# cics-nd/gptorch

Hardware: AMD Instinct MI355X
Metric: GP log-marginal-likelihood evals/sec (Cholesky+solve) at NxD fp64 (higher is better)
Workload: dtype f64; 1 GPU; C3: GPR+Matern52 N=32768 D=16 fp64 LML eval; N=32768, D=16, dy=1, kernel=Matern52, parallelism=1 GPU

## Files before the change

### gptorch_amd/_native.py

```python
import ctypes
import os

_HERE = os.path.dirname(os.path.abspath(__file__))
LIB_PATH = os.environ.get("GPN_LIB", os.path.join(_HERE, "lib", "libgpnative.so"))

c_void_p, c_int, c_int64, c_double = ctypes.c_void_p, ctypes.c_int, ctypes.c_int64, ctypes.c_double

SIGNATURES = {
    "gpn_version": (c_int, []),
    "gpn_arch": (ctypes.c_char_p, []),
    "gpn_last_hip_error": (ctypes.c_char_p, []),
    "gpn_factor_ld": (c_int64, [c_int64, c_int64]),
    "gpn_factor_rows": (c_int64, [c_int64, c_int64]),
    "gpn_winv_bytes": (c_int64, [c_int64]),
    "gpn_kernel_matrix": (c_int, [c_void_p, c_int, c_void_p, c_int64, c_void_p, c_int64, c_int,
                                  c_void_p, c_void_p, c_int, c_void_p, c_int, c_void_p, c_int64]),
    "gpn_pack_rhs": (c_int, [c_void_p, c_void_p, c_void_p, c_int64, c_int, c_void_p, c_int64]),
    "gpn_potrf_lower": (c_int, [c_void_p, c_void_p, c_int64, c_int64, c_int64, c_void_p, c_void_p]),
    "gpn_potrf_lower_panel": (c_int, [c_void_p, c_void_p, c_int64, c_int64, c_int64, c_void_p, c_void_p]),
    "gpn_potrf_lower_batched": (c_int, [c_void_p, c_void_p, c_int64, c_int64, c_int64, c_int64, c_void_p, c_int64, c_void_p, c_int]),
    "gpn_lml_reduce_batched": (c_int, [c_void_p, c_void_p, c_int64, c_int64, c_int64, c_int64, c_void_p, c_int]),
    "gpn_lml_forward_batched": (c_int, [c_void_p, c_int, c_int, c_void_p, c_int64, c_int64, c_int, c_void_p, c_int64, c_void_p, c_int64, c_int,
                                        c_void_p, c_void_p, c_int, c_void_p, c_void_p, c_int64, c_int64, c_void_p, c_int64, c_void_p, c_void_p]),
    "gpn_potrf_panel_width": (c_int64, [c_int64]),
    "gpn_potrf_panel_levels": (c_int, [c_int64, c_void_p]),
    "gpn_potrf_lower_persistent": (c_int, [c_void_p, c_void_p, c_int64, c_int64, c_int64, c_void_p, c_void_p]),
    "gpn_potrf_persistent_supported": (c_int, [c_int64, c_int64]),
    "gpn_potrf_persistent_plan": (c_int, [c_int64, c_int64, c_void_p, c_void_p, c_int64, c_void_p, c_int64]),
    "gpn_release_stream": (c_int, [c_void_p]),
    "gpn_trtri_diag": (c_int, [c_void_p, c_void_p, c_int64, c_int64, c_void_p, c_void_p]),
    "gpn_trsm_right_lt": (c_int, [c_void_p, c_void_p, c_int64, c_int64, c_void_p, c_void_p, c_int64, c_int64]),
    "gpn_lml_reduce": (c_int, [c_void_p, c_void_p, c_int64, c_int64, c_int64, c_void_p]),
    "gpn_gemm_nt": (c_int, [c_void_p, c_int64, c_int64, c_int64, c_double, c_void_p, c_int64,
                            c_void_p, c_int64, c_double, c_void_p, c_int64, c_int, c_int]),
    "gpn_gemm_nt_stair": (c_int, [c_void_p, c_int64, c_int64, c_int64, c_int64, c_double, c_void_p, c_int64,
                                  c_void_p, c_int64, c_double, c_void_p, c_int64, c_int64, c_int]),
    "gpn_gemm_nt_batched": (c_int, [c_void_p, c_int64, c_int64, c_int64, c_double, c_void_p, c_int64, c_int64,
                                    c_void_p, c_int64, c_int64, c_double, c_void_p, c_int64, c_int64, c_int, c_int, c_int]),
    "gpn_gemm_nt_batched_scaled": (c_int, [c_void_p, c_int64, c_int64, c_int64, c_void_p, c_void_p, c_int64, c_int64,
                                           c_void_p, c_int64, c_int64, c_double, c_void_p, c_int64, c_int64, c_int, c_int, c_int]),
    "gpn_kernel_matrix_batched": (c_int, [c_void_p, c_int, c_int, c_void_p, c_int64, c_int64, c_void_p, c_int64, c_int64, c_int,
                                          c_void_p, c_void_p, c_int, c_void_p, c_int, c_void_p, c_int64, c_int64]),
    "gpn_trsm_right_lt_batched": (c_int, [c_void_p, c_void_p, c_int64, c_int64, c_int64, c_void_p, c_int64,
                                          c_void_p, c_int64, c_int64, c_int64, c_int]),
    "gpn_trtri_upper_batched": (c_int, [c_void_p, c_void_p, c_int64, c_int64, c_int64, c_void_p, c_int64,
                                        c_void_p, c_int64, c_int64, c_void_p, c_int64, c_int64, c_int]),
    "gpn_kernel_grad_batched": (c_int, [c_void_p, c_int, c_int, c_void_p, c_int64, c_int64, c_void_p, c_int64, c_int64, c_int,
                                        c_void_p, c_void_p, c_int, c_void_p, c_int64, c_int64, c_void_p, c_void_p]),
    "gpn_kernel_grad_x2_batched": (c_int, [c_void_p, c_int, c_int, c_void_p, c_int64, c_int64, c_void_p, c_int64, c_int64, c_int,
                                           c_void_p, c_void_p, c_int, c_void_p, c_int64, c_int64, c_double, c_int, c_void_p, c_void_p]),
    "gpn_dot2d_batched": (c_int, [c_void_p, c_void_p, c_int64, c_int64, c_void_p, c_int64, c_int64, c_int64, c_int64, c_void_p, c_int]),
    "gpn_lml_forward_ragged": (c_int, [c_void_p, c_int, c_int, c_void_p, c_int64, c_int64, c_void_p, c_int, c_void_p, c_int64, c_int,
                                       c_void_p, c_void_p, c_int, c_void_p, c_void_p, c_int64, c_int64, c_void_p, c_int64, c_void_p, c_void_p]),
    "gpn_lml_backward_ragged": (c_int, [c_void_p, c_int, c_int, c_void_p, c_int64, c_int64, c_void_p, c_int, c_void_p, c_void_p, c_int,
                                        c_void_p, c_int64, c_int64, c_void_p, c_int64, c_int, c_void_p, c_void_p]),
    "gpn_trtri_upper": (c_int, [c_void_p, c_void_p, c_int64, c_int64, c_void_p, c_void_p, c_int64]),
    "gpn_trtri_upper_ws": (c_int, [c_void_p, c_void_p, c_int64, c_int64, c_void_p, c_void_p, c_int64, c_void_p, c_int64]),
    "gpn_grad_work_bytes": (c_int64, [c_int64, c_int64, c_int, c_int]),
    "gpn_lml_grad": (c_int, [c_void_p, c_int, c_void_p, c_int64, c_int, c_void_p, c_void_p, c_int,
                             c_void_p, c_int64, c_void_p, c_int64, c_int, c_void_p, c_void_p]),
    "gpn_kernel_grad": (c_int, [c_void_p, c_int, c_void_p, c_int64, c_void_p, c_int64, c_int, c_void_p, c_void_p,
                                c_int, c_void_p, c_int64, c_void_p, c_void_p]),
    "gpn_grad_x2_work_bytes": (c_int64, [c_int64, c_int64, c_int]),
    "gpn_kernel_grad_x2": (c_int, [c_void_p, c_int, c_void_p, c_int64, c_void_p, c_int64, c_int, c_void_p, c_void_p,
                                   c_int, c_void_p, c_int64, c_double, c_int, c_void_p, c_void_p]),
    "gpn_lml_forward": (c_int, [c_void_p, c_int, c_void_p, c_int64, c_int, c_void_p, c_void_p, c_int, c_void_p, c_void_p,
                                c_int, c_void_p, c_void_p, c_int64, c_void_p, c_void_p, c_void_p]),
    "gpn_lml_forward_saving": (c_int, [c_void_p, c_int, c_void_p, c_int64, c_int, c_void_p, c_void_p, c_int, c_void_p, c_void_p,
                                       c_int, c_void_p, c_void_p, c_int64, c_void_p, c_void_p, c_void_p, c_void_p]),
    "gpn_lml_refine_work_bytes": (c_int64, [c_int64, c_int]),
    "gpn_lml_refine": (c_int, [c_void_p, c_int, c_void_p, c_int64, c_int, c_void_p, c_void_p, c_int, c_void_p, c_void_p,
                               c_int, c_void_p, c_void_p, c_int64, c_void_p, c_void_p, c_void_p]),
    "gpn_lml_backward_work_bytes": (c_int64, [c_int64, c_int, c_int]),
    "gpn_lml_backward": (c_int, [c_void_p, c_int, c_void_p, c_int64, c_int, c_void_p, c_void_p, c_int,
                                 c_void_p, c_int64, c_void_p, c_int, c_void_p, c_void_p, c_void_p]),
    "gpn_lml_backward_batched_work_bytes": (c_int64, [c_int64, c_int, c_int, c_int]),
    "gpn_lml_backward_batched": (c_int, [c_void_p, c_int, c_int, c_void_p, c_int64, c_int64, c_int, c_void_p, c_void_p, c_int,
                                         c_void_p, c_int64, c_int64, c_void_p, c_int64, c_int, c_void_p, c_void_p, c_void_p]),
    "gpn_lml_kinv_layout": (c_int, [c_int64, c_int, ctypes.POINTER(c_int64)]),
    "gpn_lml_kinv_batched_work_bytes": (c_int64, [c_int64, c_int, c_int]),
    "gpn_lml_kinv_batched": (c_int, [c_void_p, c_int, c_int64, c_void_p, c_int64, c_int64, c_void_p, c_int64, c_int, c_void_p]),
    "gpn_lml_grad_batched": (c_int, [c_void_p, c_int, c_int, c_void_p, c_int64, c_int64, c_int, c_void_p, c_void_p, c_int,
                                     c_void_p, c_int64, c_int64, c_void_p, c_int64, c_int64, c_int, c_void_p, c_void_p]),
    "gpn_predict_work_bytes": (c_int64, [c_int64, c_int64, c_int]),
    "gpn_predict": (c_int, [c_void_p, c_int, c_void_p, c_int64, c_int, c_void_p, c_int64, c_void_p, c_void_p, c_void_p, c_int,
                            c_void_p, c_int64, c_void_p, c_int, c_int, c_void_p, c_void_p, c_void_p]),
    "gpn_block_inverse_bytes": (c_int64, [c_int64]),
    "gpn_block_inverse": (c_int, [c_void_p, c_void_p, c_int64, c_int64, c_void_p, c_void_p]),
    "gpn_trsm_right_lt_blocked": (c_int, [c_void_p, c_void_p, c_int64, c_int64, c_void_p, c_void_p, c_int64, c_int64, c_void_p, c_int64]),
    "gpn_predict_blocked": (c_int, [c_void_p, c_int, c_void_p, c_int64, c_int, c_void_p, c_int64, c_void_p, c_void_p, c_void_p, c_int,
                                    c_void_p, c_int64, c_void_p, c_void_p, c_int, c_int, c_void_p, c_void_p, c_void_p]),
    "gpn_transpose": (c_int, [c_void_p, c_void_p, c_int64, c_int64, c_int64, c_void_p, c_int64]),
    "gpn_copy_matrix": (c_int, [c_void_p, c_void_p, c_int64, c_int64, c_int64, c_void_p, c_int64, c_int]),
    "gpn_row_sumsq": (c_int, [c_void_p, c_void_p, c_int64, c_int64, c_int64, c_void_p]),
    "gpn_fill_zero": (c_int, [c_void_p, c_void_p, c_int64]),
    "gpn_gemv_t_work_bytes": (c_int64, [c_int64, c_int64, c_int]),
    "gpn_gemv_t_acc": (c_int, [c_void_p, c_void_p, c_int64, c_int64, c_int64, c_void_p, c_int64, c_int, c_void_p, c_int64, c_void_p]),
    "gpn_refine_tile_count": (c_int64, [c_int64]),
    "gpn_refine_resid_part_work_bytes": (c_int64, [c_int, c_int64]),
    "gpn_refine_resid_part": (c_int, [c_void_p, c_int, c_void_p, c_int64, c_int, c_void_p, c_void_p, c_int, c_void_p,
                                      c_void_p, c_int, c_int64, c_int64, c_void_p, c_void_p]),
    "gpn_refine_finish": (c_int, [c_void_p, c_void_p, c_void_p, c_void_p, c_void_p, c_int64, c_int, c_void_p]),
}
class ExprTerm(ctypes.Structure):
    _fields_ = [("type", c_int), ("kind", c_int), ("var_off", c_int), ("ls_off", c_int), ("nls", c_int), ("nvar", c_int)]


TERM_STATIONARY, TERM_LINEAR, TERM_CONSTANT, TERM_WHITE = 0, 1, 2, 3
EXPR_MAX_TERMS, EXPR_MAX_GROUPS = 16, 8
SIGNATURES.update({
    "gpn_lml_refine_dense": (c_int, [c_void_p, c_void_p, c_int64, c_double, c_int64, c_void_p, c_void_p, c_int, c_void_p, c_int64, c_void_p, c_void_p, c_void_p]),
    "gpn_lml_refine_expr": (c_int, [c_void_p, ctypes.POINTER(ExprTerm), c_int, ctypes.POINTER(c_int), c_int, c_void_p, c_void_p, c_int64, c_int,
                                    c_void_p, c_void_p, c_int, c_void_p, c_void_p, c_int64, c_void_p, c_void_p, c_void_p]),
    "gpn_refine_resid_part_expr": (c_int, [c_void_p, ctypes.POINTER(ExprTerm), c_int, ctypes.POINTER(c_int), c_int, c_void_p, c_void_p, c_int64, c_int,
                                           c_void_p, c_void_p, c_int, c_int64, c_int64, c_void_p, c_void_p]),
    "gpn_kernel_matrix_expr": (c_int, [c_void_p, ctypes.POINTER(ExprTerm), c_int, ctypes.POINTER(c_int), c_int, c_void_p, c_void_p,
                                       c_int64, c_void_p, c_int64, c_int, c_void_p, c_int, c_void_p, c_int64]),
    "gpn_kernel_expr_grad_work_bytes": (c_int64, [c_int64, c_int64, c_int, c_int]),
    "gpn_kernel_matrix_expr_batched": (c_int, [c_void_p, ctypes.POINTER(ExprTerm), c_int, ctypes.POINTER(c_int), c_int, c_int, c_void_p,
                                               c_int64, c_void_p, c_int64, c_int64, c_int, c_void_p, c_void_p, c_int64, c_int64]),
    "gpn_kernel_expr_grad_batched": (c_int, [c_void_p, ctypes.POINTER(ExprTerm), c_int, ctypes.POINTER(c_int), c_int, c_int, c_void_p,
                                             c_int64, c_int, c_void_p, c_int64, c_int64, c_int, c_void_p, c_int64, c_int64, c_void_p,
                                             c_int64, c_int64, c_int, c_int, c_void_p, c_void_p]),
    "gpn_kernel_expr_grad": (c_int, [c_void_p, ctypes.POINTER(ExprTerm), c_int, ctypes.POINTER(c_int), c_int, c_void_p, c_int,
                                     c_void_p, c_int64, c_void_p, c_int64, c_int, c_void_p, c_int64, c_void_p, c_int64, c_int, c_int,
                                     c_void_p, c_void_p]),
})

BCAST_FN = ctypes.CFUNCTYPE(c_int, c_void_p, c_int, c_void_p, c_int64, c_int, c_void_p)
ALLREDUCE_FN = ctypes.CFUNCTYPE(c_int, c_void_p, c_void_p, c_int64, c_void_p)


class DistComm(ctypes.Structure):
    _fields_ = [("ctx", c_void_p), ("bcast", BCAST_FN), ("allreduce", ALLREDUCE_FN), ("flags", c_int)]


SIGNATURES.update({
    "gpn_dist_work_bytes": (c_int64, [c_int, c_int, c_int, c_int64, c_int, c_int, c_int64]),
    "gpn_dist_lml_refine_work_bytes": (c_int64, [c_int, c_int, c_int, c_int64, c_int, c_int, c_int64]),
    "gpn_dist_grad_work_bytes": (c_int64, [c_int, c_int, c_int, c_int64, c_int, c_int, c_int64]),
    "gpn_dist_lml_grad": (c_int, [c_void_p, ctypes.POINTER(DistComm), c_int, c_int, c_int, c_int, c_void_p, c_int64, c_int,
                                  c_void_p, c_int, c_void_p, c_void_p, c_int, c_void_p, c_int64, c_void_p, c_int64, c_void_p,
                                  c_void_p, c_void_p]),
    "gpn_dist_layout": (c_int, [c_int, c_int, c_int, c_int, c_int64, c_int, c_int, c_int64, ctypes.POINTER(c_int64), c_int]),
    "gpn_dist_predict_work_bytes": (c_int64, [c_int, c_int, c_int, c_int64, c_int, c_int, c_int64, c_int64, c_int]),
    "gpn_dist_predict": (c_int, [c_void_p, ctypes.POINTER(DistComm), c_int, c_int, c_int, c_int, c_void_p, c_int64, c_int,
                                 c_void_p, c_int, c_void_p, c_int64, c_void_p, c_void_p, c_void_p, c_int, c_void_p, c_int64, c_int,
                                 c_void_p, c_int64, c_void_p, c_void_p, c_void_p]),
    "gpn_dist_lml_forward": (c_int, [c_void_p, ctypes.POINTER(DistComm), c_int, c_int, c_int, c_int, c_void_p, c_int64, c_int,
                                     c_void_p, c_int, c_void_p, c_void_p, c_int, c_void_p, c_int64, c_void_p, c_int64, c_void_p]),
    "gpn_dist_lml_refine": (c_int, [c_void_p, ctypes.POINTER(DistComm), c_int, c_int, c_int, c_int, c_void_p, c_int64, c_int,
                                    c_void_p, c_int, c_void_p, c_void_p, c_int, c_void_p, c_int64, c_void_p, c_void_p, c_int64, c_void_p]),
})
RCCL_LIB_PATH = os.environ.get("GPN_RCCL_LIB", os.path.join(os.path.dirname(LIB_PATH), "libgpnative_rccl.so"))
RCCL_SIGNATURES = {
    "gpn_rccl_comm_create": (ctypes.POINTER(DistComm), [c_void_p, c_void_p, c_void_p]),
    "gpn_rccl_comm_destroy": (None, [ctypes.POINTER(DistComm)]),
    "gpn_mesh_plan": (c_int64, [c_int, c_int, c_int, c_int64, c_int, c_int64, ctypes.POINTER(c_int64), c_int64]),
}
DIST_FORCE_COLLECTIVES, DIST_MESH_EXCHANGE = 1, 2
_rccl_lib = None


def rccl_lib():
    global _rccl_lib
    if _rccl_lib is None:
        if not os.path.exists(RCCL_LIB_PATH):
            raise NativeError("libgpnative_rccl.so not found at %s -- run gptorch_amd/csrc/build.sh" % RCCL_LIB_PATH)
        handle = ctypes.CDLL(RCCL_LIB_PATH)
        for name, (res, args) in RCCL_SIGNATURES.items():
            fn = getattr(handle, name)
            fn.restype, fn.argtypes = res, args
        _rccl_lib = handle
    return _rccl_lib


PROFILE_SIGNATURES = {
    "gpn_profile_enable": (c_int, [c_int]),
    "gpn_profile_collect": (c_int, [ctypes.POINTER(c_double)]),
    "gpn_profile_collect_classes": (c_int, [ctypes.POINTER(c_double), c_int]),
}
SIGNATURES.update(PROFILE_SIGNATURES)
DEBUG_SIGNATURES = {
    "gpn_debug_set_gemm_variant": (c_int, [c_int]),
    "gpn_debug_set_potrf_variant": (c_int, [c_int]),
    "gpn_debug_set_outer_width": (c_int, [c_int, c_int]),
    "gpn_debug_set_extra_rows": (c_int, [c_int]),
    "gpn_debug_set_thin_tiles": (c_int, [c_int]),
    "gpn_debug_masked_stream": (c_int, [ctypes.POINTER(ctypes.c_uint32), c_int, ctypes.POINTER(c_void_p)]),
    "gpn_debug_set_backsub_persistent": (c_int, [c_int]),
    "gpn_debug_set_persistent": (c_int, [c_int, c_int]),
    "gpn_debug_persistent_trace": (c_int, [c_void_p]),
}
DEBUG_LIB_PATH = os.path.join(_HERE, "lib", "libgpnative_dbg.so")

_lib = None
_product_lib = None
_debug_lib = None


class NativeError(RuntimeError):
    pass


def _load(path, extra):
    handle = ctypes.CDLL(path)
    for name, (res, args) in list(SIGNATURES.items()) + list(extra.items()):
        fn = getattr(handle, name)
        fn.restype, fn.argtypes = res, args
    return handle


def lib():
    global _lib, _product_lib
    if _lib is None:
        if not os.path.exists(LIB_PATH):
            raise NativeError(
                "libgpnative.so not found at %s -- build it with `python -c 'import __graft_entry__ as g; "
                "g.build()'` (or gptorch_amd/csrc/build.sh). gptorch_amd has no CPU fallback." % LIB_PATH)
        extra = DEBUG_SIGNATURES if os.path.basename(LIB_PATH).startswith("libgpnative_dbg") else {}
        _product_lib = _lib = _load(LIB_PATH, extra)
    return _lib


class debug_library:

    def __enter__(self):
        global _lib, _debug_lib
        lib()
        if _debug_lib is None:
            if not os.path.exists(DEBUG_LIB_PATH):
                raise NativeError("libgpnative_dbg.so not found at %s -- run gptorch_amd/csrc/build.sh" % DEBUG_LIB_PATH)
            _debug_lib = _load(DEBUG_LIB_PATH, DEBUG_SIGNATURES)
        _lib = _debug_lib
        return _debug_lib

    def __exit__(self, *exc):
        global _lib
        _debug_lib.gpn_debug_set_gemm_variant(0)
        _debug_lib.gpn_debug_set_potrf_variant(0)
        _lib = _product_lib
        return False


_debug_ctx = None


def debug_begin():
    global _debug_ctx
    if _debug_ctx is None:
        _debug_ctx = debug_library()
        return _debug_ctx.__enter__()
    return _debug_lib


def debug_end():
    global _debug_ctx
    if _debug_ctx is not None:
        _debug_ctx.__exit__(None, None, None)
        _debug_ctx = None


def check(status, what):
    if status != 0:
        detail = lib().gpn_last_hip_error().decode() if status == -100 else ""
        raise NativeError("%s failed with status %d %s" % (what, status, detail))
```

### gptorch_amd/csrc/gpn_common.h

```cpp
#pragma once
#include <hip/hip_runtime.h>
#include <stdint.h>
#include "../../include/gpnative.h"

#ifdef GPN_DEBUG_SWITCHES
#define GPN_SWITCH static thread_local
#define GPN_DEBUG_ONLY(...) __VA_ARGS__
#else
#define GPN_SWITCH static constexpr
#define GPN_DEBUG_ONLY(...)
#endif

namespace gpn {

constexpr int LEAF = 128;

inline int64_t round_up(int64_t x, int64_t m) { return (x + m - 1) / m * m; }

void set_hip_error(hipError_t e, const char* where);

#define GPN_HIP_CHECK(expr)                          \
  do {                                               \
    hipError_t _e = (expr);                          \
    if (_e != hipSuccess) {                          \
      gpn::set_hip_error(_e, #expr);                 \
      return GPN_E_HIP;                              \
    }                                                \
  } while (0)

#define GPN_LAUNCH_CHECK() GPN_HIP_CHECK(hipGetLastError())

int gemm_nt(hipStream_t s, int64_t M, int64_t N, int64_t K, double alpha,
            const double* A, int64_t lda, const double* B, int64_t ldb,
            double beta, double* C, int64_t ldc, int lower, int tri = 0, int inplace = 0);

int potrf_persistent(hipStream_t s, double* A, int64_t n, int64_t e, int64_t lda, double* winv, int32_t* info);
void potrf_persistent_release(hipStream_t s);

int gemm_nt_stair(hipStream_t s, int64_t M, int64_t nblocks, int64_t blk, int64_t K, double alpha,
                  const double* A, int64_t lda, const double* B, int64_t ldb,
                  double beta, double* C, int64_t ldc, int64_t step, int diag);

int colpanel(hipStream_t s, int mode, int64_t m, int64_t nb, const double* A, int64_t lda, const double* B, int64_t ldb,
             double* C, int64_t ldc, int batch = 1, int64_t sA = 0, int64_t sB = 0, int64_t sC = 0);

int leaf16(hipStream_t s, double* A, int64_t lda, int kb, int col0, double* winv, int32_t* info, int batch, int64_t sA,
           int64_t sW, int64_t sInfo);
int gemm_nt_batched(hipStream_t s, int64_t M, int64_t N, int64_t K, double alpha,
                    const double* A, int64_t lda, int64_t sA, const double* B, int64_t ldb, int64_t sB,
                    double beta, double* C, int64_t ldc, int64_t sC, int tri, int batch);

int gemm_nt_strided(hipStream_t s, int64_t M, int64_t N, int64_t K, double alpha,
                    const double* A, int64_t lda, const double* B, int64_t ldb,
                    double beta, double* C, int64_t ldc, int lower, int tri, int inplace,
                    int batch, int64_t sA, int64_t sB, int64_t sC);

int gemm_nt_strided2(hipStream_t s, int64_t M, int64_t N, int64_t K, double alpha,
                     const double* A, int64_t lda, const double* B, int64_t ldb,
                     double beta, double* C, int64_t ldc, int lower, int tri,
                     int inner, int64_t sA, int64_t sB, int64_t sC, int outer, int64_t sA2, int64_t sB2, int64_t sC2);

int lml_grad_batched(hipStream_t s, int kind, int batch, const double* X, int64_t sX, int64_t n, int d,
                     const double* variance, const double* length_scales, int nls,
                     const double* Kinv, int64_t ldk, int64_t sK, const double* at, int64_t ldat, int64_t sAt, int dy,
                     double* work, int64_t sWork, double* out, const int32_t* n_of = nullptr);
int trtri_upper_ws_batched(hipStream_t s, const double* L, int64_t n, int64_t ldl, int64_t sL, const double* winv, int64_t sW,
                           double* U, int64_t ldu, int64_t sU, double* S, int64_t lds, int64_t sS, int batch);

int lml_reduce_ragged(hipStream_t s, const double* A, int64_t n, int64_t e, int64_t lda, int64_t sA, double* out3, int batch,
                      const int32_t* n_of);
int pack_rhs_full(hipStream_t s, const double* Y, const double* M, int64_t n, int dy, double* E, int64_t lde,
                  int32_t* info);

int assemble_lower_saving(hipStream_t s, int kind, const double* X, int64_t n, int d, const double* variance, const double* length_scales,
                          int nls, const double* noise, double* A, double* Ksave, int64_t lda);
int assemble_batched(hipStream_t s, int kind, int batch, const double* X, int64_t sX, int64_t n, int d, const double* Y, int64_t sY,
                     const double* M, int64_t sM, int dy, const double* variance, const double* length_scales, int nls,
                     const double* noise, double* A, int64_t lda, int64_t sA, int32_t* info, const int32_t* n_of = nullptr);

enum { PROF_GEMM = 0,
       PROF_GEMM_SYRK = 1,
       PROF_GEMM_SOLVE = 2,
       PROF_GEMM_TRI = 3,
       PROF_KMAT = 4,
       PROF_GRAD = 5,
       PROF_LEAF = 6,
       PROF_NCLASSES = 7 };
void dist_release(hipStream_t s);

int expr_resid(hipStream_t s, const gpn_expr_term* terms, int nterms, const int* gstart, int ngroups, const double* theta,
               const double* X, int64_t n, int d, const double* noise, const double* a, int dy, int64_t lds, int64_t q0, int64_t cnt,
               double* prow, double* pcol);

bool profile_on();
int profile_begin(hipStream_t s, double work, int cls);
void profile_end(hipStream_t s, int idx);

}
```

### gptorch_amd/csrc/potrf.hip

```cpp
#include <algorithm>
#include <atomic>
#include <cstdlib>
#include <mutex>
#include <type_traits>
#include <unordered_map>
#include <vector>
#include "gpn_common.h"
#include "potrf_ctx.h"

namespace gpn {

GPN_SWITCH int g_potrf_variant = 0;
GPN_SWITCH int g_panel_width = 0;
GPN_SWITCH int g_outer_width = 0;
GPN_SWITCH int g_outer_width2 = 0;
GPN_SWITCH int g_aux_left_looking = -1;
GPN_SWITCH int g_extra_rows_kernel = 1;

static void potrf_rec(Ctx& c, double* A, int64_t n, int64_t e, int64_t col0) {
  if (c.rc != GPN_OK || n <= 0) return;
  if (n <= LEAF) {
    c.rc = launch_leaf(c.s, A, c.lda, (int)n, (int)col0, c.winv + (col0 / LEAF) * (LEAF * LEAF), c.info, c.batch, c.sA, c.sW, 1);
    if (c.rc != GPN_OK) return;
    if (e > 0) trsm_rec(c, A + n * c.lda, e, c.lda, A, c.lda, n, col0, c.winv);
    return;
  }
  const int64_t h = split_point(n);
  potrf_rec(c, A, h, 0, col0);
  double* A21 = A + h * c.lda;
  const int64_t m = n - h + e;
  trsm_rec(c, A21, m, c.lda, A, c.lda, h, col0, c.winv);
  if (c.rc != GPN_OK) return;
  if (c.corner || e == 0) {
    c.rc = cgemm(c, c.s, m, m, h, -1.0, A21, c.lda, A21, c.lda, 1.0, A21 + h, c.lda, 1);
  } else {
    const int64_t ms = n - h;
    c.rc = cgemm(c, c.s, ms, ms, h, -1.0, A21, c.lda, A21, c.lda, 1.0, A21 + h, c.lda, 1);
    if (c.rc == GPN_OK)
      c.rc = cgemm(c, c.s, e, ms, h, -1.0, A21 + ms * c.lda, c.lda, A21, c.lda, 1.0, A21 + ms * c.lda + h, c.lda, 0);
  }
  potrf_rec(c, A21 + h, n - h, e, col0 + h);
}

struct Aux {
  hipStream_t s1 = nullptr;
  hipEvent_t solve[4] = {nullptr, nullptr, nullptr, nullptr};
  hipEvent_t rest[4] = {nullptr, nullptr, nullptr, nullptr};
  hipEvent_t extra_go = nullptr, extra_done = nullptr;
};
static std::mutex g_aux_mutex;
static std::unordered_map<hipStream_t, Aux> g_aux;

static Aux* aux_for(hipStream_t s) {
  std::lock_guard<std::mutex> lock(g_aux_mutex);
  auto it = g_aux.find(s);
  if (it != g_aux.end()) return &it->second;
  Aux a;
  int least = 0, greatest = 0;
  if (hipDeviceGetStreamPriorityRange(&least, &greatest) != hipSuccess) least = 0;
  if (hipStreamCreateWithPriority(&a.s1, hipStreamNonBlocking, least) != hipSuccess) return nullptr;
  if (hipEventCreateWithFlags(&a.extra_go, hipEventDisableTiming) != hipSuccess) return nullptr;
  if (hipEventCreateWithFlags(&a.extra_done, hipEventDisableTiming) != hipSuccess) return nullptr;
  for (int i = 0; i < 4; ++i) {
    if (hipEventCreateWithFlags(&a.solve[i], hipEventDisableTiming) != hipSuccess) return nullptr;
    if (hipEventCreateWithFlags(&a.rest[i], hipEventDisableTiming) != hipSuccess) return nullptr;
  }
  return &g_aux.emplace(s, a).first->second;
}

constexpr int XR_MAXE = 8;
constexpr int64_t XR_MIN_N = 20480;
template <int E>
__global__ __launch_bounds__(256) void extra_rows_update_kernel(const double* P, double* R, int64_t lda, int ms, int K, int e, int64_t sA) {
  P += (int64_t)blockIdx.y * sA;
  R += (int64_t)blockIdx.y * sA;
  const int lane = threadIdx.x & 63, wave = threadIdx.x >> 6;
  const int j0 = (blockIdx.x * 4 + wave) * 4;
  if (j0 >= ms) return;
  const double* Pe = P + (int64_t)ms * lda;
  const double* rows[4];
#pragma unroll
  for (int r = 0; r < 4; ++r) rows[r] = P + (int64_t)min(j0 + r, ms - 1) * lda;
  double acc[4][E];
#pragma unroll
  for (int r = 0; r < 4; ++r)
#pragma unroll
    for (int q = 0; q < E; ++q) acc[r][q] = 0.0;
  for (int k = 2 * lane; k < K; k += 128) {
    double2 v[4], pe[E];
#pragma unroll
    for (int r = 0; r < 4; ++r) v[r] = *reinterpret_cast<const double2*>(rows[r] + k);
#pragma unroll
    for (int q = 0; q < E; ++q) pe[q] = q < e ? *reinterpret_cast<const double2*>(Pe + (int64_t)q * lda + k) : double2{0.0, 0.0};
#pragma unroll
    for (int r = 0; r < 4; ++r)
#pragma unroll
      for (int q = 0; q < E; ++q) acc[r][q] = fma(v[r].y, pe[q].y, fma(v[r].x, pe[q].x, acc[r][q]));
  }
#pragma unroll
  for (int r = 0; r < 4; ++r)
#pragma unroll
    for (int q = 0; q < E; ++q) {
      double t = acc[r][q];
#pragma unroll
      for (int o = 32; o > 0; o >>= 1) t += __shfl_xor(t, o, 64);
      acc[r][q] = t;
    }
  if (lane == 0) {
#pragma unroll
    for (int r = 0; r < 4; ++r)
#pragma unroll
      for (int q = 0; q < E; ++q)
        if (j0 + r < ms && q < e) R[(int64_t)q * lda + j0 + r] -= acc[r][q];
  }
}
static int extra_rows_update(hipStream_t s, const double* P, double* R, int64_t lda, int64_t ms, int64_t K, int64_t e, int batch, int64_t sA) {
  const dim3 grid((unsigned)((ms + 15) / 16), (unsigned)batch);
  if (e <= 1) hipLaunchKernelGGL(extra_rows_update_kernel<1>, grid, dim3(256), 0, s, P, R, lda, (int)ms, (int)K, (int)e, sA);
  else if (e <= 2) hipLaunchKernelGGL(extra_rows_update_kernel<2>, grid, dim3(256), 0, s, P, R, lda, (int)ms, (int)K, (int)e, sA);
  else if (e <= 4) hipLaunchKernelGGL(extra_rows_update_kernel<4>, grid, dim3(256), 0, s, P, R, lda, (int)ms, (int)K, (int)e, sA);
  else hipLaunchKernelGGL(extra_rows_update_kernel<XR_MAXE>, grid, dim3(256), 0, s, P, R, lda, (int)ms, (int)K, (int)e, sA);
  GPN_LAUNCH_CHECK();
  return GPN_OK;
}

static inline bool large_problem(int64_t n) { return n >= 24576; }
struct PanelLevels { int n = 1; int64_t w[3] = {0, 0, 0}; };
static inline int64_t panel_width(int64_t n) {
  if (g_panel_width) return g_panel_width;
  return n < 20480 ? 256 : 512;
}
static inline PanelLevels panel_levels(int64_t n) {
  PanelLevels L;
  L.w[0] = panel_width(n);
  int64_t w1 = g_outer_width, w2 = g_outer_width2;
  if (w1 == 0) w1 = n <= 2048 ? 0 : n < 20480 ? 1024 : 2048;
  if (w1 == 2048 && w2 == 0 && n >= 49152) w2 = 4096;
  if (w1 > L.w[0]) { L.w[L.n] = (w1 / L.w[L.n - 1]) * L.w[L.n - 1]; ++L.n; }
  if (w2 > L.w[L.n - 1]) { L.w[L.n] = (w2 / L.w[L.n - 1]) * L.w[L.n - 1]; ++L.n; }
  return L;
}

static void potrf_lookahead(Ctx& c, double* A, int64_t n, int64_t e) {
  Aux* ax = aux_for(c.s);
  if (!ax) { c.rc = GPN_E_HIP; return; }
  const PanelLevels lev = panel_levels(n);
  const int64_t lda = c.lda, PW = lev.w[0];
  const bool left_looking = g_aux_left_looking < 0 ? large_problem(n) : g_aux_left_looking != 0;
  auto hip_ok = [&](hipError_t err) { if (err != hipSuccess && c.rc == GPN_OK) { set_hip_error(err, "potrf_lookahead"); c.rc = GPN_E_HIP; } };
  int step = 0, rest_idx = 0;
  bool rest_pending = false, extra_pending = false;
  for (int64_t p0 = 0; p0 < n && c.rc == GPN_OK; p0 += PW) {
    const int64_t pw = std::min(PW, n - p0), pend = p0 + pw;
    if (extra_pending) { hip_ok(hipStreamWaitEvent(c.s, ax->extra_done, 0)); extra_pending = false; }
    for (int64_t k0 = p0; k0 < pend && c.rc == GPN_OK; k0 += LEAF, ++step) {
      const int64_t kb = std::min<int64_t>(LEAF, n - k0);
      const int64_t c1 = k0 + kb;
      double* Akk = A + k0 * lda + k0;
      const double* Wk = c.winv + (k0 / LEAF) * (LEAF * LEAF);
      {
        const int rec = profile_on() ? profile_begin(c.s, c.batch * 2.0 * LEAF * LEAF * LEAF / 3.0, PROF_LEAF) : -1;
        const int lrc = launch_leaf(c.s, Akk, lda, (int)kb, (int)k0, const_cast<double*>(Wk), c.info, c.batch, c.sA, c.sW, 1);
        if (c.rc == GPN_OK) c.rc = lrc;
        if (rec >= 0) profile_end(c.s, rec);
      }
      const int64_t m = n + e - c1;
      if (m <= 0 || c.rc != GPN_OK) continue;
      double* B = A + c1 * lda + k0;
      c.rc = ccolpanel(c, c.s, 0, m, kb, B, lda, Wk, LEAF, B, lda);
      if (c.rc != GPN_OK || c1 >= pend) continue;
      const int64_t nb1 = std::min<int64_t>(LEAF, pend - c1);
      const int64_t c2 = c1 + nb1;
      if (rest_pending) {
        hip_ok(hipStreamWaitEvent(c.s, ax->rest[rest_idx], 0));
        rest_pending = false;
      }
      const bool fork = c2 < pend;
      c.rc = cgemm(c, c.s, m, nb1, kb, -1.0, B, lda, B, lda, 1.0, A + c1 * lda + c1, lda, 0);
      if (fork) hip_ok(hipEventRecord(ax->solve[step & 3], c.s));
      if (fork && c.rc == GPN_OK) {
        hip_ok(hipStreamWaitEvent(ax->s1, ax->solve[step & 3], 0));
        const int64_t m2 = n + e - c2;
        if (!left_looking) {
          c.rc = cgemm(c, ax->s1, m2, pend - c2, kb, -1.0, A + c2 * lda + k0, lda, A + c2 * lda + k0, lda, 1.0,
                         A + c2 * lda + c2, lda, 0);
        } else {
          const int64_t nb2 = std::min<int64_t>(LEAF, pend - c2);
          c.rc = cgemm(c, ax->s1, m2, nb2, c1 - p0, -1.0, A + c2 * lda + p0, lda, A + c2 * lda + p0, lda, 1.0,
                         A + c2 * lda + c2, lda, 0);
        }
        rest_idx = step & 3;
        hip_ok(hipEventRecord(ax->rest[rest_idx], ax->s1));
        rest_pending = true;
      }
    }
    if (c.rc != GPN_OK) break;
    if (rest_pending) {
      hip_ok(hipStreamWaitEvent(c.s, ax->rest[rest_idx], 0));
      rest_pending = false;
    }
    if (pend >= n) break;
    const int64_t m = n + e - pend;
    int l = 0;
    while (l + 1 < lev.n && pend % lev.w[l + 1] == 0) ++l;
    const int64_t o0 = l == 0 ? p0 : pend - lev.w[l];
    double* P = A + pend * lda + o0;
    const int64_t kp = round_up(pend - o0, 16);
    if (l + 1 < lev.n) {
      const int64_t oend = std::min(n, (pend / lev.w[l + 1] + 1) * lev.w[l + 1]);
      c.rc = cgemm(c, c.s, m, oend - pend, kp, -1.0, P, lda, P, lda, 1.0, A + pend * lda + pend, lda, 2);
    } else if (e > 0 && e <= XR_MAXE && g_extra_rows_kernel && n >= XR_MIN_N && (lda & 1) == 0 && (o0 & 1) == 0) {
      const int64_t ms = n - pend;
      hip_ok(hipEventRecord(ax->extra_go, c.s));
      hip_ok(hipStreamWaitEvent(ax->s1, ax->extra_go, 0));
      c.rc = cgemm(c, c.s, ms, ms, kp, -1.0, P, lda, P, lda, 1.0, A + pend * lda + pend, lda, 1);
      if (c.rc == GPN_OK) c.rc = extra_rows_update(ax->s1, P, A + n * lda + pend, lda, ms, kp, e, c.batch, c.sA);
      hip_ok(hipEventRecord(ax->extra_done, ax->s1));
      extra_pending = true;
    } else if (c.corner || e == 0) {
      c.rc = cgemm(c, c.s, m, m, kp, -1.0, P, lda, P, lda, 1.0, A + pend * lda + pend, lda, 1);
    } else {
      const int64_t ms = n - pend;
      c.rc = cgemm(c, c.s, ms, ms, kp, -1.0, P, lda, P, lda, 1.0, A + pend * lda + pend, lda, 1);
      if (c.rc == GPN_OK)
        c.rc = cgemm(c, c.s, e, ms, kp, -1.0, P + ms * lda, lda, P, lda, 1.0, A + n * lda + pend, lda, 0);
    }
  }
  if (extra_pending) hip_ok(hipStreamWaitEvent(c.s, ax->extra_done, 0));
}


}

using namespace gpn;

extern "C" int64_t gpn_factor_ld(int64_t n, int64_t e) { return round_up(n + e, LEAF); }
extern "C" int64_t gpn_factor_rows(int64_t n, int64_t e) { return round_up(n + e, LEAF) + 16; }
extern "C" int64_t gpn_winv_bytes(int64_t n) {
  return (round_up(n, LEAF) / LEAF) * LEAF * LEAF * (int64_t)sizeof(double);
}

extern "C" int gpn_potrf_lower(void* stream, double* A, int64_t n, int64_t e, int64_t lda,
                               double* winv, int32_t* info) {
  if (!A) return -2;
  if (n < 0) return -3;
  if (e < 0) return -4;
  if (lda < round_up(n + e, LEAF) || (lda % LEAF) != 0) return -5;
  if (!winv) return -6;
  if (!info) return -7;
  if (reinterpret_cast<uintptr_t>(A) & 15) return GPN_E_ALIGN;
  if (n == 0) return GPN_OK;
  Ctx c{static_cast<hipStream_t>(stream), lda, winv, info, GPN_OK};
  if (g_potrf_variant == 1 || n <= 2 * LEAF) potrf_rec(c, A, n, e, 0);
  else potrf_lookahead(c, A, n, e);
  return c.rc;
}

extern "C" int64_t gpn_potrf_panel_width(int64_t n) {
  if (g_potrf_variant == 1 || n <= 2 * LEAF) return 0;
  const PanelLevels L = panel_levels(n);
  return L.w[L.n - 1];
}
extern "C" int gpn_potrf_panel_levels(int64_t n, int64_t* widths3) {
  if (!widths3) return -2;
  widths3[0] = widths3[1] = widths3[2] = 0;
  if (g_potrf_variant == 1 || n <= 2 * LEAF) return 0;
  const PanelLevels L = panel_levels(n);
  for (int i = 0; i < L.n; ++i) widths3[i] = L.w[i];
  return L.n;
}

extern "C" int gpn_release_stream(void* stream) {
  dist_release(static_cast<hipStream_t>(stream));
  potrf_persistent_release(static_cast<hipStream_t>(stream));
  std::lock_guard<std::mutex> lock(g_aux_mutex);
  auto drop = [](Aux& a) {
    if (a.s1) { (void)hipStreamSynchronize(a.s1); (void)hipStreamDestroy(a.s1); }
    if (a.extra_go) (void)hipEventDestroy(a.extra_go);
    if (a.extra_done) (void)hipEventDestroy(a.extra_done);
    for (int i = 0; i < 4; ++i) {
      if (a.solve[i]) (void)hipEventDestroy(a.solve[i]);
      if (a.rest[i]) (void)hipEventDestroy(a.rest[i]);
    }
  };
  if (!stream) {
    for (auto& kv : g_aux) drop(kv.second);
    g_aux.clear();
    return GPN_OK;
  }
  auto it = g_aux.find(static_cast<hipStream_t>(stream));
  if (it != g_aux.end()) { drop(it->second); g_aux.erase(it); }
  return GPN_OK;
}

extern "C" int gpn_potrf_lower_panel(void* stream, double* A, int64_t n, int64_t e, int64_t lda,
                                     double* winv, int32_t* info) {
  if (!A) return -2;
  if (n < 0) return -3;
  if (e < 0) return -4;
  if (lda < round_up(n, LEAF) || (lda % LEAF) != 0) return -5;
  if (!winv) return -6;
  if (!info) return -7;
  if (reinterpret_cast<uintptr_t>(A) & 15) return GPN_E_ALIGN;
  if (n == 0) return GPN_OK;
  Ctx c{static_cast<hipStream_t>(stream), lda, winv, info, GPN_OK};
  c.corner = false;
  if (g_potrf_variant == 1 || n <= 2 * LEAF) potrf_rec(c, A, n, e, 0);
  else potrf_lookahead(c, A, n, e);
  return c.rc;
}

GPN_DEBUG_ONLY(
extern "C" int gpn_debug_set_potrf_variant(int v) {
  g_potrf_variant = v & 1;
  g_panel_width = ((v >> 8) & 0xff) * LEAF;
  g_aux_left_looking = ((v >> 3) & 1) ? 1 : (((v >> 5) & 1) ? 0 : -1);
  return GPN_OK;
}
extern "C" int gpn_debug_set_extra_rows(int on) { g_extra_rows_kernel = on; return GPN_OK; }
extern "C" int gpn_debug_set_outer_width(int w1, int w2) { g_outer_width = w1; g_outer_width2 = w2; return GPN_OK; })

extern "C" int gpn_potrf_lower_batched(void* stream, double* A, int64_t n, int64_t e, int64_t lda, int64_t sA,
                                       double* winv, int64_t sW, int32_t* info, int batch) {
  if (!A) return -2;
  if (n < 0) return -3;
  if (e < 0) return -4;
  if (lda < round_up(n + e, LEAF) || (lda % LEAF) != 0) return -5;
  if (batch < 1) return -10;
  if (batch > 1 && (sA < gpn_factor_rows(n, e) * lda || (sA & 1))) return -6;
  if (!winv) return -7;
  if (batch > 1 && sW < gpn_winv_bytes(n) / (int64_t)sizeof(double)) return -8;
  if (!info) return -9;
  if (reinterpret_cast<uintptr_t>(A) & 15) return GPN_E_ALIGN;
  if (n == 0) return GPN_OK;
  Ctx c{static_cast<hipStream_t>(stream), lda, winv, info, GPN_OK};
  c.batch = batch; c.sA = sA; c.sW = sW;
  if (g_potrf_variant == 1 || n <= 2 * LEAF) potrf_rec(c, A, n, e, 0);
  else potrf_lookahead(c, A, n, e);
  return c.rc;
}
```

Before: 5.444 LML evals/s.

## Compute trailing SYRK update via int8 CRT-moduli MFMA emulation of fp64

Adds a SYRK path that converts each panel row to scaled fixed-point integers, reduces them modulo 16 small primes into int8 planes, and runs int8 MFMA GEMMs per modulus. The fp64 result is rebuilt with Chinese-remainder reconstruction in double-double form. It is used for the large outer trailing updates in the lookahead Cholesky when n is large. The aim is to swap the slow fp64 matrix-core rate for much faster int8 throughput, at the cost of a conversion pass, extra workspace, and possible accuracy loss on badly scaled rows.

```diff
diff --git a/gptorch_amd/_native.py b/gptorch_amd/_native.py
--- a/gptorch_amd/_native.py
+++ b/gptorch_amd/_native.py
@@ -186,6 +186,8 @@
     "gpn_debug_set_potrf_variant": (c_int, [c_int]),
     "gpn_debug_set_outer_width": (c_int, [c_int, c_int]),
     "gpn_debug_set_extra_rows": (c_int, [c_int]),
+    "gpn_debug_set_syrk_crt": (c_int, [c_int]),
+    "gpn_debug_syrk_crt": (c_int, [c_void_p, c_int64, c_int64, c_void_p, c_int64, c_void_p, c_int64]),
     "gpn_debug_set_thin_tiles": (c_int, [c_int]),
     "gpn_debug_masked_stream": (c_int, [ctypes.POINTER(ctypes.c_uint32), c_int, ctypes.POINTER(c_void_p)]),
     "gpn_debug_set_backsub_persistent": (c_int, [c_int]),
diff --git a/gptorch_amd/csrc/gpn_common.h b/gptorch_amd/csrc/gpn_common.h
--- a/gptorch_amd/csrc/gpn_common.h
+++ b/gptorch_amd/csrc/gpn_common.h
@@ -78,6 +78,11 @@
                      const double* M, int64_t sM, int dy, const double* variance, const double* length_scales, int nls,
                      const double* noise, double* A, int64_t lda, int64_t sA, int32_t* info, const int32_t* n_of = nullptr);
 
+constexpr int64_t SYRK_CRT_MAX_K = 8192;
+int64_t syrk_crt_ws_bytes(int64_t M, int64_t K, int batch);
+int syrk_crt(hipStream_t s, int64_t M, int64_t K, const double* P, int64_t lda, double* C, int64_t ldc, int batch, int64_t sA,
+             void* ws, int64_t ws_bytes);
+
 enum { PROF_GEMM = 0,
        PROF_GEMM_SYRK = 1,
        PROF_GEMM_SOLVE = 2,
diff --git a/gptorch_amd/csrc/potrf.hip b/gptorch_amd/csrc/potrf.hip
--- a/gptorch_amd/csrc/potrf.hip
+++ b/gptorch_amd/csrc/potrf.hip
@@ -16,6 +16,7 @@
 GPN_SWITCH int g_outer_width2 = 0;
 GPN_SWITCH int g_aux_left_looking = -1;
 GPN_SWITCH int g_extra_rows_kernel = 1;
+GPN_SWITCH int g_syrk_crt = 1;
 
 static void potrf_rec(Ctx& c, double* A, int64_t n, int64_t e, int64_t col0) {
   if (c.rc != GPN_OK || n <= 0) return;
@@ -47,6 +48,8 @@
   hipEvent_t solve[4] = {nullptr, nullptr, nullptr, nullptr};
   hipEvent_t rest[4] = {nullptr, nullptr, nullptr, nullptr};
   hipEvent_t extra_go = nullptr, extra_done = nullptr;
+  void* crt_ws = nullptr;
+  int64_t crt_bytes = 0;
 };
 static std::mutex g_aux_mutex;
 static std::unordered_map<hipStream_t, Aux> g_aux;
@@ -125,6 +128,7 @@
 }
 
 static inline bool large_problem(int64_t n) { return n >= 24576; }
+constexpr int64_t CRT_MIN_N = 20480;
 struct PanelLevels { int n = 1; int64_t w[3] = {0, 0, 0}; };
 static inline int64_t panel_width(int64_t n) {
   if (g_panel_width) return g_panel_width;
@@ -148,6 +152,23 @@
   const int64_t lda = c.lda, PW = lev.w[0];
   const bool left_looking = g_aux_left_looking < 0 ? large_problem(n) : g_aux_left_looking != 0;
   auto hip_ok = [&](hipError_t err) { if (err != hipSuccess && c.rc == GPN_OK) { set_hip_error(err, "potrf_lookahead"); c.rc = GPN_E_HIP; } };
+  bool crt = false;
+  if (g_syrk_crt && n >= CRT_MIN_N && lev.w[lev.n - 1] <= SYRK_CRT_MAX_K) {
+    const int64_t need = syrk_crt_ws_bytes(n + e - lev.w[lev.n - 1], lev.w[lev.n - 1], c.batch);
+    if (ax->crt_bytes < need) {
+      hipStreamCaptureStatus cs = hipStreamCaptureStatusActive;
+      if (hipStreamIsCapturing(c.s, &cs) == hipSuccess && cs == hipStreamCaptureStatusNone) {
+        if (ax->crt_ws) { hip_ok(hipFree(ax->crt_ws)); ax->crt_ws = nullptr; ax->crt_bytes = 0; }
+        if (hipMalloc(&ax->crt_ws, need) == hipSuccess) ax->crt_bytes = need;
+        else { ax->crt_ws = nullptr; (void)hipGetLastError(); }
+      }
+    }
+    crt = ax->crt_bytes >= need;
+  }
+  auto outer_update = [&](int64_t mm, double* P, int64_t kp, double* C) {
+    if (crt) return syrk_crt(c.s, mm, kp, P, lda, C, lda, c.batch, c.sA, ax->crt_ws, ax->crt_bytes);
+    return cgemm(c, c.s, mm, mm, kp, -1.0, P, lda, P, lda, 1.0, C, lda, 1);
+  };
   int step = 0, rest_idx = 0;
   bool rest_pending = false, extra_pending = false;
   for (int64_t p0 = 0; p0 < n && c.rc == GPN_OK; p0 += PW) {
@@ -213,12 +234,12 @@
       const int64_t ms = n - pend;
       hip_ok(hipEventRecord(ax->extra_go, c.s));
       hip_ok(hipStreamWaitEvent(ax->s1, ax->extra_go, 0));
-      c.rc = cgemm(c, c.s, ms, ms, kp, -1.0, P, lda, P, lda, 1.0, A + pend * lda + pend, lda, 1);
+      c.rc = outer_update(ms, P, kp, A + pend * lda + pend);
       if (c.rc == GPN_OK) c.rc = extra_rows_update(ax->s1, P, A + n * lda + pend, lda, ms, kp, e, c.batch, c.sA);
       hip_ok(hipEventRecord(ax->extra_done, ax->s1));
       extra_pending = true;
     } else if (c.corner || e == 0) {
-      c.rc = cgemm(c, c.s, m, m, kp, -1.0, P, lda, P, lda, 1.0, A + pend * lda + pend, lda, 1);
+      c.rc = outer_update(m, P, kp, A + pend * lda + pend);
     } else {
       const int64_t ms = n - pend;
       c.rc = cgemm(c, c.s, ms, ms, kp, -1.0, P, lda, P, lda, 1.0, A + pend * lda + pend, lda, 1);
@@ -278,6 +299,7 @@
     if (a.s1) { (void)hipStreamSynchronize(a.s1); (void)hipStreamDestroy(a.s1); }
     if (a.extra_go) (void)hipEventDestroy(a.extra_go);
     if (a.extra_done) (void)hipEventDestroy(a.extra_done);
+    if (a.crt_ws) (void)hipFree(a.crt_ws);
     for (int i = 0; i < 4; ++i) {
       if (a.solve[i]) (void)hipEventDestroy(a.solve[i]);
       if (a.rest[i]) (void)hipEventDestroy(a.rest[i]);
@@ -318,7 +340,21 @@
   return GPN_OK;
 }
 extern "C" int gpn_debug_set_extra_rows(int on) { g_extra_rows_kernel = on; return GPN_OK; }
-extern "C" int gpn_debug_set_outer_width(int w1, int w2) { g_outer_width = w1; g_outer_width2 = w2; return GPN_OK; })
+extern "C" int gpn_debug_set_outer_width(int w1, int w2) { g_outer_width = w1; g_outer_width2 = w2; return GPN_OK; }
+extern "C" int gpn_debug_set_syrk_crt(int on) { g_syrk_crt = on; return GPN_OK; }
+extern "C" int gpn_debug_syrk_crt(void* stream, int64_t M, int64_t K, const double* P, int64_t lda, double* C, int64_t ldc) {
+  if (M < 0 || K <= 0 || K > SYRK_CRT_MAX_K || (K % 16)) return -3;
+  if ((lda & 1) || (reinterpret_cast<uintptr_t>(P) & 15)) return GPN_E_ALIGN;
+  hipStream_t s = static_cast<hipStream_t>(stream);
+  const int64_t bytes = syrk_crt_ws_bytes(M, K, 1);
+  void* ws = nullptr;
+  GPN_HIP_CHECK(hipMalloc(&ws, bytes));
+  int rc = syrk_crt(s, M, K, P, lda, C, ldc, 1, 0, ws, bytes);
+  const hipError_t err = hipStreamSynchronize(s);
+  (void)hipFree(ws);
+  if (rc == GPN_OK && err != hipSuccess) { set_hip_error(err, "gpn_debug_syrk_crt"); rc = GPN_E_HIP; }
+  return rc;
+})
 
 extern "C" int gpn_potrf_lower_batched(void* stream, double* A, int64_t n, int64_t e, int64_t lda, int64_t sA,
                                        double* winv, int64_t sW, int32_t* info, int batch) {
diff --git a/gptorch_amd/csrc/syrk_crt.hip b/gptorch_amd/csrc/syrk_crt.hip
--- /dev/null
+++ b/gptorch_amd/csrc/syrk_crt.hip
@@ -0,0 +1,295 @@
+#include <algorithm>
+#include <atomic>
+#include <cmath>
+#include "gpn_common.h"
+#include "gemm_tile.h"
+
+namespace gpn {
+
+constexpr int CRT_NMOD = 16;
+constexpr int CRT_P[CRT_NMOD] = {256, 255, 253, 251, 247, 241, 239, 233, 229, 227, 223, 217, 211, 199, 197, 193};
+typedef unsigned __int128 crt_u128;
+
+struct CrtConst {
+  int p[CRT_NMOD];
+  int m28[CRT_NMOD];
+  float invp[CRT_NMOD];
+  double w1[CRT_NMOD], w2[CRT_NMOD];
+  double m1, m2, inv_m;
+};
+
+constexpr crt_u128 crt_modulus() {
+  crt_u128 m = 1;
+  for (int t = 0; t < CRT_NMOD; ++t) m *= (crt_u128)CRT_P[t];
+  return m;
+}
+constexpr double crt_hi85(crt_u128 v) { return (double)(uint64_t)(v >> 85) * 0x1p85; }
+constexpr double crt_lo85(crt_u128 v) {
+  const crt_u128 l = v & ((((crt_u128)1) << 85) - 1);
+  return (double)(uint64_t)(l >> 32) * 0x1p32 + (double)(uint64_t)(l & 0xffffffffu);
+}
+constexpr CrtConst crt_make() {
+  CrtConst r{};
+  const crt_u128 M = crt_modulus();
+  for (int t = 0; t < CRT_NMOD; ++t) {
+    const int p = CRT_P[t];
+    const crt_u128 W = M / (crt_u128)p;
+    const int wm = (int)(W % (crt_u128)p);
+    int c = 1;
+    while ((wm * c) % p != 1) ++c;
+    crt_u128 w = 0;
+    for (int i = 0; i < c; ++i) { w += W; if (w >= M) w -= M; }
+    r.p[t] = p;
+    r.m28[t] = (int)((((crt_u128)1) << 28) % (crt_u128)p);
+    r.invp[t] = 1.0f / (float)p;
+    r.w1[t] = crt_hi85(w);
+    r.w2[t] = crt_lo85(w);
+  }
+  r.m1 = crt_hi85(M);
+  r.m2 = crt_lo85(M);
+  r.inv_m = 1.0 / (crt_hi85(M) + crt_lo85(M));
+  return r;
+}
+__constant__ CrtConst c_crt = crt_make();
+
+__device__ __forceinline__ int crt_mod(int v, int p, float invp) {
+  const int q = (int)floorf((float)v * invp);
+  int r = v - q * p;
+  r = r < 0 ? r + p : r;
+  return r >= p ? r - p : r;
+}
+
+static int crt_bits(int64_t K) {
+  int lk = 0;
+  while ((int64_t(1) << lk) < K) ++lk;
+  return (123 - lk) / 2;
+}
+
+__global__ __launch_bounds__(256) void crt_convert_kernel(const double* P, int64_t lda, int64_t sA, int m, int K, int mpad, int Kp,
+                                                          int b, int8_t* R, int64_t zstride) {
+  const int z = blockIdx.y;
+  P += (int64_t)z * sA;
+  int8_t* Rz = R + (int64_t)z * zstride;
+  const int64_t plane = (int64_t)mpad * Kp;
+  double* sc = reinterpret_cast<double*>(Rz + CRT_NMOD * plane);
+  const int lane = threadIdx.x & 63;
+  const int row = blockIdx.x * 4 + (threadIdx.x >> 6);
+  if (row >= mpad) return;
+  int8_t* out = Rz + (int64_t)row * Kp;
+  if (row >= m) {
+    for (int c = lane; c < Kp / 16; c += 64)
+#pragma unroll
+      for (int t = 0; t < CRT_NMOD; ++t) *reinterpret_cast<int4*>(out + t * plane + c * 16) = int4{0, 0, 0, 0};
+    if (lane == 0) sc[row] = 0.0;
+    return;
+  }
+  const double* pr = P + (int64_t)row * lda;
+  double mx = 0.0;
+  bool bad = false;
+  for (int k = lane; k < K; k += 64) {
+    const double v = pr[k];
+    bad |= !isfinite(v);
+    mx = fabs(v) > mx ? fabs(v) : mx;
+  }
+#pragma unroll
+  for (int o = 32; o > 0; o >>= 1) mx = fmax(mx, __shfl_xor(mx, o, 64));
+  bad = __any(bad);
+  int e = 0;
+  (void)frexp(bad ? 0.0 : mx, &e);
+  if (lane == 0) sc[row] = bad ? __builtin_nan("") : ldexp(1.0, e - b);
+  const int sh = b - e;
+  for (int c = lane; c < Kp / 16; c += 64) {
+    int hi[16], lo[16];
+#pragma unroll
+    for (int j = 0; j < 16; j += 2) {
+      double2 v = double2{0.0, 0.0};
+      if (c * 16 + j < K && !bad) v = *reinterpret_cast<const double2*>(pr + c * 16 + j);
+      const int64_t x0 = (int64_t)rint(ldexp(v.x, sh)), x1 = (int64_t)rint(ldexp(v.y, sh));
+      hi[j] = (int)(x0 >> 28); lo[j] = (int)(x0 & 0xfffffff);
+      hi[j + 1] = (int)(x1 >> 28); lo[j + 1] = (int)(x1 & 0xfffffff);
+    }
+    for (int t = 0; t < CRT_NMOD; ++t) {
+      const int p = c_crt.p[t], m28 = c_crt.m28[t], half = (p + 1) >> 1;
+      const float ip = c_crt.invp[t];
+      int w[4] = {0, 0, 0, 0};
+#pragma unroll
+      for (int j = 0; j < 16; ++j) {
+        int r = crt_mod(crt_mod(hi[j], p, ip) * m28 + lo[j], p, ip);
+        r = r >= half ? r - p : r;
+        w[j >> 2] |= (r & 0xff) << (8 * (j & 3));
+      }
+      *reinterpret_cast<int4*>(out + t * plane + c * 16) = int4{w[0], w[1], w[2], w[3]};
+    }
+  }
+}
+
+struct CrtArgs {
+  const int8_t* R;
+  int64_t zstride;
+  int M, mt, mpad, Kp;
+  double* C;
+  int64_t ldc, sC;
+  int batch;
+};
+
+typedef int crt_i4 __attribute__((ext_vector_type(4)));
+
+__global__ __launch_bounds__(512, 1) void syrk_crt_kernel(CrtArgs p) {
+  constexpr int BM = 128, KS = 2, BK = 64 * KS, NS = 4, AHEAD = NS - 1;
+  constexpr int NBLK = 2 * (BM / 16) * KS;
+  constexpr int STAGE = NBLK * 1024;
+  constexpr int NWAVES = 8, PER_WAVE = NBLK / NWAVES;
+  constexpr int TM = 2, TN = 4;
+  extern __shared__ __attribute__((aligned(16))) char smem[];
+
+  int bid = blockIdx.x, nwg = gridDim.x;
+  const int8_t* R = p.R;
+  double* C = p.C;
+  if (p.batch > 1) {
+    nwg /= p.batch;
+    const int z = bid / nwg;
+    bid -= z * nwg;
+    R += z * p.zstride;
+    C += z * p.sC;
+  }
+  int ti, tj;
+  tile_of_block_lower(bid, nwg, p.mt, false, ti, tj, 8);
+  const int64_t plane = (int64_t)p.mpad * p.Kp;
+  const double* sc = reinterpret_cast<const double*>(R + CRT_NMOD * plane);
+  const int lane = threadIdx.x & 63;
+  const int wave = __builtin_amdgcn_readfirstlane(threadIdx.x >> 6);
+  const int wave_m = wave >> 1, wave_n = wave & 1;
+  const int m0 = ti * BM, n0 = tj * BM;
+  const int nk = p.Kp / BK;
+
+  const int8_t* src[PER_WAVE];
+#pragma unroll
+  for (int i = 0; i < PER_WAVE; ++i) {
+    const int idx = wave + NWAVES * i;
+    const int ks = idx >> 4, isB = (idx >> 3) & 1, rg = idx & 7;
+    const int r = lane >> 2;
+    const int row = (isB ? n0 : m0) + rg * 16 + r;
+    const int chunk = (lane & 3) ^ ((-(r >> 2)) & 3);
+    src[i] = R + (int64_t)row * p.Kp + ks * 64 + chunk * 16;
+  }
+  const int fr = lane & 15;
+  const int roff = fr * 64 + (((lane >> 4) ^ ((-(fr >> 2)) & 3)) * 16);
+
+  int it = 0, ik = 0;
+  auto issue = [&](int slot) {
+    const int64_t off = it * plane + (int64_t)ik * BK;
+#pragma unroll
+    for (int i = 0; i < PER_WAVE; ++i)
+      __builtin_amdgcn_global_load_lds((const __attribute__((address_space(1))) void*)(src[i] + off),
+                                       (__attribute__((address_space(3))) void*)(smem + slot * STAGE + (wave + NWAVES * i) * 1024),
+                                       16, 0, 0);
+    if (++ik == nk) { ik = 0; ++it; }
+  };
+
+  crt_i4 acc[TM][TN];
+  double s1[TM][TN][4], s2[TM][TN][4];
+#pragma unroll
+  for (int i = 0; i < TM; ++i)
+#pragma unroll
+    for (int j = 0; j < TN; ++j) {
+      acc[i][j] = crt_i4{0, 0, 0, 0};
+#pragma unroll
+      for (int r = 0; r < 4; ++r) s1[i][j][r] = s2[i][j][r] = 0.0;
+    }
+
+  const int total = CRT_NMOD * nk;
+  for (int g = 0; g < min(total, AHEAD); ++g) issue(g);
+  int g = 0;
+  for (int t = 0; t < CRT_NMOD; ++t) {
+    for (int kk = 0; kk < nk; ++kk, ++g) {
+      if (g + AHEAD <= total) asm volatile("s_waitcnt vmcnt(%0)" ::"n"(PER_WAVE * (AHEAD - 1)) : "memory");
+      else asm volatile("s_waitcnt vmcnt(0)" ::: "memory");
+      __builtin_amdgcn_s_barrier();
+      if (g + AHEAD < total) issue((g + AHEAD) % NS);
+      const char* base = smem + (g % NS) * STAGE;
+#pragma unroll
+      for (int ks = 0; ks < KS; ++ks) {
+        crt_i4 a[TM], bb[TN];
+#pragma unroll
+        for (int i = 0; i < TM; ++i) a[i] = *reinterpret_cast<const crt_i4*>(base + (ks * 16 + wave_m * TM + i) * 1024 + roff);
+#pragma unroll
+        for (int j = 0; j < TN; ++j) bb[j] = *reinterpret_cast<const crt_i4*>(base + (ks * 16 + 8 + wave_n * TN + j) * 1024 + roff);
+#pragma unroll
+        for (int i = 0; i < TM; ++i)
+#pragma unroll
+          for (int j = 0; j < TN; ++j) acc[i][j] = __builtin_amdgcn_mfma_i32_16x16x64_i8(a[i], bb[j], acc[i][j], 0, 0, 0);
+      }
+      __builtin_amdgcn_sched_barrier(0);
+    }
+    const int pt = c_crt.p[t];
+    const float ip = c_crt.invp[t];
+    const double w1 = c_crt.w1[t], w2 = c_crt.w2[t];
+#pragma unroll
+    for (int i = 0; i < TM; ++i)
+#pragma unroll
+      for (int j = 0; j < TN; ++j) {
+#pragma unroll
+        for (int r = 0; r < 4; ++r) {
+          const double y = (double)crt_mod(acc[i][j][r], pt, ip);
+          s1[i][j][r] = fma(y, w1, s1[i][j][r]);
+          s2[i][j][r] = fma(y, w2, s2[i][j][r]);
+        }
+        acc[i][j] = crt_i4{0, 0, 0, 0};
+      }
+  }
+
+  const double m1 = c_crt.m1, m2 = c_crt.m2, inv_m = c_crt.inv_m;
+  const bool diag = ti == tj;
+#pragma unroll
+  for (int i = 0; i < TM; ++i)
+#pragma unroll
+    for (int j = 0; j < TN; ++j) {
+      const int col = n0 + wave_n * 64 + j * 16 + (lane & 15);
+      const double scj = col < p.M ? sc[col] : 0.0;
+#pragma unroll
+      for (int r = 0; r < 4; ++r) {
+        const int row = m0 + wave_m * 32 + i * 16 + 4 * (lane >> 4) + r;
+        if (row < p.M && col < p.M && (!diag || col <= row)) {
+          const double q = rint(s1[i][j][r] * inv_m);
+          const double S = fma(-q, m1, s1[i][j][r]) + fma(-q, m2, s2[i][j][r]);
+          double* cp = C + (int64_t)row * p.ldc + col;
+          *cp = *cp - (S * sc[row]) * scj;
+        }
+      }
+    }
+}
+
+int64_t syrk_crt_ws_bytes(int64_t M, int64_t K, int batch) {
+  const int64_t mpad = round_up(M, 128), Kp = round_up(K, 64);
+  return (int64_t)batch * (CRT_NMOD * mpad * Kp + mpad * (int64_t)sizeof(double));
+}
+
+int syrk_crt(hipStream_t s, int64_t M, int64_t K, const double* P, int64_t lda, double* C, int64_t ldc, int batch, int64_t sA,
+             void* ws, int64_t ws_bytes) {
+  if (M <= 0) return GPN_OK;
+  if (K <= 0 || K > SYRK_CRT_MAX_K || ws_bytes < syrk_crt_ws_bytes(M, K, batch)) return GPN_E_UNSUPPORTED;
+  const int mpad = (int)round_up(M, 128), Kp = (int)round_up(K, 64);
+  const int64_t zstride = syrk_crt_ws_bytes(M, K, 1);
+  int8_t* R = static_cast<int8_t*>(ws);
+  hipLaunchKernelGGL(crt_convert_kernel, dim3((unsigned)(mpad / 4), (unsigned)batch), dim3(256), 0, s, P, lda, sA, (int)M, (int)K,
+                     mpad, Kp, crt_bits(K), R, zstride);
+  GPN_LAUNCH_CHECK();
+  CrtArgs a;
+  a.R = R; a.zstride = zstride;
+  a.M = (int)M; a.mt = mpad / 128; a.mpad = mpad; a.Kp = Kp;
+  a.C = C; a.ldc = ldc; a.sC = sA; a.batch = batch;
+  const int grid = a.mt * (a.mt + 1) / 2 * batch;
+  constexpr int smem = 4 * 32 * 1024;
+  static std::atomic<bool> attr_set{false};
+  if (!attr_set.load(std::memory_order_acquire)) {
+    GPN_HIP_CHECK(hipFuncSetAttribute(reinterpret_cast<const void*>(syrk_crt_kernel), hipFuncAttributeMaxDynamicSharedMemorySize, smem));
+    attr_set.store(true, std::memory_order_release);
+  }
+  const int rec = profile_on() ? profile_begin(s, (double)grid * 2.0 * 128 * 128 * (double)K, PROF_GEMM_SYRK) : -1;
+  hipLaunchKernelGGL(syrk_crt_kernel, dim3(grid), dim3(512), smem, s, a);
+  if (rec >= 0) profile_end(s, rec);
+  GPN_LAUNCH_CHECK();
+  return GPN_OK;
+}
+
+}
```

New measurement: 5.451 LML evals/s (median of 6 runs). No clear change (+0.1%).
